# AlexIoannides/bodywork-mlops-demo

Measured on NVIDIA H100. Metric: train rows/sec (N x 128 least-squares fit), higher is better.
Workload: dtype bf16x2 (hi+lo) MMA operands, f32 accumulate, f64 fold+solve

## Files before the change

bodywork-mlops-demo_b200/csrc/solve.cu:

```cuda
#include "b2_internal.cuh"
#include "b2_xchg.cuh"

namespace b2 {
namespace {

constexpr int kOutIntercept = kMaxD;
constexpr int kOutInfo = kMaxD + 1;
constexpr int kOutRank = kMaxD + 2;
constexpr int kOutSingular = kMaxD + 3;
constexpr int kOutRows = kOutSingular + kMaxD;

struct LdcgStat {
  const double* S;
  __device__ __forceinline__ double operator()(int i) const { return __ldcg(S + i); }
};

template <class Stat>
__device__ void build_normal_equations_of(const Stat& S, int d, double alpha, int fit_intercept,
                                       double* A, double* r, double* mean, double* ybar_out) {
  const int dp = d + 2, pitch = d + 1;
  const double n = S(d * dp + d);
  const double inv_n = n > 0.0 ? 1.0 / n : 0.0;
  double sxy = 0.0;
  if ((int)threadIdx.x < d) {
    const double sx = S(threadIdx.x * dp + d);
    sxy = S(threadIdx.x * dp + d + 1);
    mean[threadIdx.x] = fit_intercept ? sx * inv_n : 0.0;
  }
  const double ybar = fit_intercept ? S(d * dp + d + 1) * inv_n : 0.0;
  __syncthreads();
  if ((int)threadIdx.x < d) r[threadIdx.x] = sxy - n * mean[threadIdx.x] * ybar;
  const int lane = threadIdx.x & 31, warp = threadIdx.x >> 5, nwarps = blockDim.x >> 5;
  for (int i0 = warp; i0 < d; i0 += 2 * nwarps) {
    const int i1 = i0 + nwarps;
    double v[8];
#pragma unroll
    for (int u = 0; u < 4; ++u) {
      const int j = lane + 32 * u;
      v[u] = j < d ? S(i0 * dp + j) : 0.0;
      v[4 + u] = (j < d && i1 < d) ? S(i1 * dp + j) : 0.0;
    }
    const double m0 = mean[i0], m1 = i1 < d ? mean[i1] : 0.0;
#pragma unroll
    for (int u = 0; u < 4; ++u) {
      const int j = lane + 32 * u;
      if (j < d) {
        const double mj = mean[j];
        A[i0 * pitch + j] = v[u] - n * m0 * mj + (i0 == j ? alpha : 0.0);
        if (i1 < d) A[i1 * pitch + j] = v[4 + u] - n * m1 * mj + (i1 == j ? alpha : 0.0);
      }
    }
  }
  if (threadIdx.x == 0) *ybar_out = ybar;
  __syncthreads();
}

__device__ __forceinline__ void build_normal_equations(const double* S, int d, double alpha, int fit_intercept,
                                                       double* A, double* r, double* mean, double* ybar_out) {
  build_normal_equations_of(LdcgStat{S}, d, alpha, fit_intercept, A, r, mean, ybar_out);
}

__device__ __forceinline__ double rcp_pos(double x) {
  double y;
  asm("rcp.approx.ftz.f64 %0, %1;" : "=d"(y) : "d"(x));
  const double er = fma(-x, y, 1.0);
  const double t = fma(er, er, er);
  return fma(y, t, y);
}

struct SolveXchg {
  double* own;
  int n_ranks;
  unsigned int epoch;
  unsigned long long timeout_ns;
};

constexpr int kNB = 16;
constexpr int kCholThreads = 512;
constexpr int kUPitch = kNB + 1;

__device__ void refine_update(const double* S, int d, int fit_intercept, bool singular, const double* dbeta, double* misc,
                              double* __restrict__ rf, double* __restrict__ out);

template <bool REFINE>
__global__ void __launch_bounds__(kCholThreads, 1)
solve_cholesky_kernel(double* S, int d, double alpha, int fit_intercept, double* __restrict__ out, const SolveXchg xc,
                      double* __restrict__ rf) {
  extern __shared__ double sm[];
  const int pitch = d + 1;
  double* A = sm;
  double* r = A + d * pitch;
  double* mean = A + (d + 1) * pitch;
  double* invd = mean + d;
  double* misc = invd + d;
  double* U = misc + 8;
  const int tid = threadIdx.x, lane = tid & 31;
  const int warp = __shfl_sync(0xffffffffu, tid >> 5, 0);
  long long tm[5] = {0, 0, 0, 0, 0};
  long long tc0 = clock64();
  if (xc.own != nullptr) {
    __shared__ int ok;
    if (tid == 0) ok = xchg_wait(xc.own, xc.n_ranks, xc.epoch, xc.timeout_ns) ? 1 : 0;
    __syncthreads();
    if (!ok) {
      if (tid == 0) {
        xchg_flags(xc.own)[kXchgStatusWord] = xc.epoch;
        out[kOutInfo] = -1.0;
      }
      return;
    }
    const int dp = d + 2;
    for (int base = 0; base < dp * dp; base += 4 * blockDim.x) {
      double sv[4];
#pragma unroll
      for (int u = 0; u < 4; ++u) {
        const int idx = base + u * blockDim.x + tid;
        sv[u] = idx < dp * dp ? xchg_sum(xc.own, xc.n_ranks, xc.epoch, idx) : 0.0;
      }
#pragma unroll
      for (int u = 0; u < 4; ++u) {
        const int idx = base + u * blockDim.x + tid;
        if (idx < dp * dp) S[idx] = sv[u];
      }
    }
    __threadfence();
    __syncthreads();
  }
  build_normal_equations(S, d, alpha, fit_intercept, A, r, mean, &misc[0]);
  if constexpr (REFINE) {
    if (tid < d) r[tid] = rf[kRfGrad + tid] - alpha * rf[kRfBeta + tid];
    __syncthreads();
  }
  tm[0] = clock64() - tc0;
  if (warp == 0) {
    double mx = 0.0;
    for (int i = lane; i < d; i += 32) mx = fmax(mx, A[i * pitch + i]);
#pragma unroll
    for (int o = 16; o > 0; o >>= 1) mx = fmax(mx, __shfl_xor_sync(0xffffffffu, mx, o));
    if (lane == 0) { misc[1] = mx; misc[2] = 0.0; }
  }
  __syncthreads();
  const double tiny = misc[1] * 1e-12;
  const int rows = d + 1;

  for (int kb = 0; kb < d; kb += kNB) {
    const int nb = (d - kb) < kNB ? (d - kb) : kNB;
    tc0 = clock64();
    if (warp == 0) {
      const int lrow = lane & (kNB - 1), h = lane >> 4;
      const bool act = lrow < nb;
      const int row = kb + (act ? lrow : 0);
      double a[kNB / 2];
#pragma unroll
      for (int cc = 0; cc < kNB / 2; ++cc) {
        const int c = 2 * cc + h;
        a[cc] = (act && c < nb) ? A[row * pitch + kb + c] : 0.0;
      }
      double my_rc = 1.0;
      int first_bad = 0;
#pragma unroll
      for (int k = 0; k < kNB; ++k) {
        if (k < nb) {
          const int hk = k & 1, kk = k >> 1;
          const double colk = a[kk];
          const double piv = __shfl_sync(0xffffffffu, colk, k | (hk << 4));
          const bool bad = !(piv > tiny);
          const double rc = bad ? 1.0 : rcp_pos(piv);
          const double u = __shfl_sync(0xffffffffu, colk, lrow | (hk << 4));
          my_rc = (lrow == k) ? rc : my_rc;
          first_bad = (bad && first_bad == 0) ? (kb + k + 1) : first_bad;
#pragma unroll
          for (int cc = 0; cc < kNB / 2; ++cc) {
            if (2 * cc + 1 > k) {
              const int c = 2 * cc + h;
              const double uc = __shfl_sync(0xffffffffu, colk, c | (hk << 4));
              if (c > k) a[cc] = fma(-(u * uc), rc, a[cc]);
            }
          }
          if (h == hk && act && lrow > k) {
            A[row * pitch + kb + k] = u * rc;
            U[row * kUPitch + k] = u;
          }
        }
      }
      if (act && h == 0) invd[kb + lrow] = my_rc;
      if (lane == 0 && first_bad != 0 && misc[2] == 0.0) misc[2] = (double)first_bad;
    }
    __syncthreads();
    tm[1] += clock64() - tc0; tc0 = clock64();
    if (misc[2] != 0.0) break;
    {
      const int prow = tid >> 2, q = tid & 3;
      const int below = rows - kb - nb;
      const bool live = prow < below;
      const int i = kb + nb + (live ? prow : 0);
      double sv[4];
#pragma unroll
      for (int j = 0; j < 4; ++j) {
        const int c = 4 * j + q;
        sv[j] = (live && c < nb) ? A[i * pitch + kb + c] : 0.0;
      }
      const int qbase = lane & ~3;
      double rinv[kNB];
#pragma unroll
      for (int m = 0; m < kNB; ++m) rinv[m] = m < nb ? invd[kb + m] : 0.0;
      double out_m[4], out_u[4];
#pragma unroll
      for (int j = 0; j < 4; ++j) { out_m[j] = 0.0; out_u[j] = 0.0; }
#pragma unroll
      for (int m = 0; m < kNB; ++m) {
        if (m < nb) {
          const double um = __shfl_sync(0xffffffffu, sv[m >> 2], qbase | (m & 3));
          const double xm = um * rinv[m];
          if (q == (m & 3)) { out_m[m >> 2] = xm; out_u[m >> 2] = um; }
#pragma unroll
          for (int j = 0; j < 4; ++j) {
            if (4 * j + 3 > m) {
              const int c = 4 * j + q;
              if (c > m && c < nb) sv[j] = fma(-xm, U[(kb + c) * kUPitch + m], sv[j]);
            }
          }
        }
      }
      if (live) {
#pragma unroll
        for (int j = 0; j < 4; ++j) {
          const int m = 4 * j + q;
          if (m < nb) { A[i * pitch + kb + m] = out_m[j]; U[i * kUPitch + m] = out_u[j]; }
        }
      }
    }
    __syncthreads();
    tm[2] += clock64() - tc0; tc0 = clock64();
    {
      const int base = kb + nb;
      const int nti = (rows - base + 7) >> 3, ntj = (d - base + 7) >> 3;
      const int tri = ntj * (ntj + 1) / 2;
      const int total = tri + (nti > ntj ? ntj : 0);
      const int g = lane >> 2, t4 = lane & 3;
      constexpr int kWarps = kCholThreads / 32, kInFlight = 4;
      for (int t0 = warp; t0 < total; t0 += kWarps * kInFlight) {
        int ia[kInFlight], jb[kInFlight];
        double c0[kInFlight], c1[kInFlight], av[kInFlight][kNB / 4], bv[kInFlight][kNB / 4];
#pragma unroll
        for (int f = 0; f < kInFlight; ++f) {
          const int t = t0 + f * kWarps;
          int ti = 0, tj = 0;
          if (t < tri) {
            ti = (int)((sqrtf(8.0f * (float)t + 1.0f) - 1.0f) * 0.5f);
            while (ti * (ti + 1) / 2 > t) --ti;
            while ((ti + 1) * (ti + 2) / 2 <= t) ++ti;
            tj = t - ti * (ti + 1) / 2;
          } else if (t < total) {
            ti = ntj; tj = t - tri;
          }
          const bool live = t < total;
          ia[f] = live ? base + 8 * ti + g : rows;
          jb[f] = live ? base + 8 * tj + g : d;
#pragma unroll
          for (int sgm = 0; sgm < kNB / 4; ++sgm) {
            const int m = 4 * sgm + t4;
            av[f][sgm] = (ia[f] < rows && m < nb) ? -A[ia[f] * pitch + kb + m] : 0.0;
            bv[f][sgm] = (jb[f] < d && m < nb) ? U[jb[f] * kUPitch + m] : 0.0;
          }
          c0[f] = 0.0; c1[f] = 0.0;
        }
#pragma unroll
        for (int sgm = 0; sgm < kNB / 4; ++sgm) {
#pragma unroll
          for (int f = 0; f < kInFlight; ++f)
            asm volatile("mma.sync.aligned.m8n8k4.row.col.f64.f64.f64.f64 {%0, %1}, {%2}, {%3}, {%0, %1};"
                         : "+d"(c0[f]), "+d"(c1[f]) : "d"(av[f][sgm]), "d"(bv[f][sgm]));
        }
#pragma unroll
        for (int f = 0; f < kInFlight; ++f) {
          const int jc = jb[f] - g + 2 * t4;
          if (ia[f] < rows) {
            if (jc < d) A[ia[f] * pitch + jc] += c0[f];
            if (jc + 1 < d) A[ia[f] * pitch + jc + 1] += c1[f];
          }
        }
      }
    }
    __syncthreads();
    tm[3] += clock64() - tc0;
  }
  tc0 = clock64();
  const bool singular = misc[2] != 0.0;
  if (!singular) {
    for (int kb = ((d - 1) / kNB) * kNB; kb >= 0; kb -= kNB) {
      const int nb = (d - kb) < kNB ? (d - kb) : kNB;
      if (warp == 0) {
        const int col = lane & (kNB - 1);
        const bool act = lane < nb;
        double lt[kNB];
#pragma unroll
        for (int k = 0; k < kNB; ++k) lt[k] = (act && k < nb && k > col) ? A[(kb + k) * pitch + kb + col] : 0.0;
        double z = act ? r[kb + col] : 0.0;
#pragma unroll
        for (int k = kNB - 1; k >= 0; --k) {
          if (k < nb) {
            const double bk = __shfl_sync(0xffffffffu, z, k);
            z = (lane < k) ? fma(-lt[k], bk, z) : z;
          }
        }
        __syncwarp();
        if (act) r[kb + lane] = z;
      }
      __syncthreads();
      for (int i = tid; i < kb; i += blockDim.x) {
        double acc0 = 0.0, acc1 = 0.0;
#pragma unroll
        for (int m = 0; m < kNB; m += 2) {
          if (m < nb) acc0 = fma(A[(kb + m) * pitch + i], r[kb + m], acc0);
          if (m + 1 < nb) acc1 = fma(A[(kb + m + 1) * pitch + i], r[kb + m + 1], acc1);
        }
        r[i] -= acc0 + acc1;
      }
      __syncthreads();
    }
  }
  tm[4] = clock64() - tc0;
  if constexpr (REFINE) {
    refine_update(S, d, fit_intercept, singular, r, misc, rf, out);
    return;
  }
  if (tid == 0)
    for (int k = 0; k < 5; ++k) out[kOutSingular + k] = (double)tm[k];
  for (int i = tid; i < d; i += blockDim.x) out[i] = singular ? 0.0 : r[i];
  if (warp == 0) {
    double part = 0.0;
    for (int i = lane; i < d; i += 32) part += mean[i] * r[i];
#pragma unroll
    for (int o = 16; o > 0; o >>= 1) part += __shfl_xor_sync(0xffffffffu, part, o);
    if (lane == 0) {
      out[kOutIntercept] = singular ? 0.0 : misc[0] - part;
      out[kOutInfo] = misc[2];
    }
  }
}

__device__ void refine_update(const double* S, int d, int fit_intercept, bool singular, const double* dbeta, double* misc,
                              double* __restrict__ rf, double* __restrict__ out) {
  const int tid = threadIdx.x, lane = tid & 31, warp = tid >> 5;
  const int dp = d + 2;
  const double n = __ldcg(S + d * dp + d);
  if (warp == 0) {
    double mx = 0.0;
    bool finite = true;
    for (int i = lane; i < d; i += 32) {
      const double sx = __ldcg(S + i * dp + d);
      const double c = __ldcg(S + i * dp + i) - sx * (sx / n);
      mx = fmax(mx, fabs(dbeta[i]) * sqrt(fmax(c, 0.0)));
      finite = finite && isfinite(dbeta[i]);
    }
#pragma unroll
    for (int o = 16; o > 0; o >>= 1) mx = fmax(mx, __shfl_xor_sync(0xffffffffu, mx, o));
    finite = __all_sync(0xffffffffu, finite) && isfinite(rf[kRfGrad + kMaxD]);
    if (lane == 0) {
      const double sy = __ldcg(S + d * dp + d + 1);
      const double cy = __ldcg(S + (d + 1) * dp + d + 1) - sy * (sy / n);
      const double sig = sqrt(fmax(cy, 0.0));
      const double step = sig > 0.0 ? mx / sig : mx;
      misc[3] = step;
      misc[4] = (singular || !finite || !(step <= rf[kRfStep])) ? 1.0 : 0.0;
    }
  }
  __syncthreads();
  const bool guard = misc[4] != 0.0;
  for (int i = tid; i < d; i += blockDim.x) {
    const double b = rf[kRfBeta + i];
    if (guard) {
      rf[kRfBeta + i] = rf[kRfPrevBeta + i];
    } else {
      rf[kRfPrevBeta + i] = b;
      rf[kRfBeta + i] = b + dbeta[i];
    }
  }
  if (tid == 0) {
    const double b0 = rf[kRfB0];
    if (guard) {
      rf[kRfB0] = rf[kRfPrevB0];
    } else {
      rf[kRfPrevB0] = b0;
      rf[kRfB0] = fit_intercept ? b0 + rf[kRfGrad + kMaxD] / n : b0;
      rf[kRfStep] = misc[3];
    }
  }
  __syncthreads();
  for (int i = tid; i < d; i += blockDim.x) out[i] = rf[kRfBeta + i];
  if (warp == 0) {
    double part = 0.0;
    for (int i = lane; i < d; i += 32) part += rf[kRfMean + i] * rf[kRfBeta + i];
#pragma unroll
    for (int o = 16; o > 0; o >>= 1) part += __shfl_xor_sync(0xffffffffu, part, o);
    if (lane == 0) {
      out[kOutIntercept] = rf[kRfB0] - part;
      out[kOutInfo] = misc[2];
      out[kOutRefineStep] = misc[3];
      out[kOutRefineGuard] = misc[4];
    }
  }
}

__device__ __forceinline__ void rr_pair(int m, int round, int k, int* p, int* q) {
  const int mm = m - 1;
  int a, b;
  if (k == 0) { a = mm; b = round % mm; }
  else { a = (round + k) % mm; b = (round - k + mm) % mm; }
  *p = a < b ? a : b;
  *q = a < b ? b : a;
}

__global__ void __launch_bounds__(512, 1)
solve_spectral_kernel(const double* __restrict__ S, int d, double cond, int fit_intercept,
                      double* __restrict__ out) {
  extern __shared__ double sm[];
  const int pitch = d + 1;
  double* W = sm;
  double* r = W + d * pitch;
  double* mean = r + d;
  double* lam = mean + d;
  double* misc = lam + d;
  __shared__ int rotated;
  build_normal_equations(S, d, 0.0, fit_intercept, W, r, mean, &misc[0]);

  const int m = d + (d & 1);
  const int pairs = m / 2;
  const int sub = threadIdx.x & 7;
  const int slot0 = threadIdx.x >> 3;
  for (int sweep = 0; sweep < 24 && d > 1; ++sweep) {
    if (threadIdx.x == 0) rotated = 0;
    __syncthreads();
    for (int round = 0; round < m - 1; ++round) {
      for (int slot = slot0; slot < ((pairs + 63) / 64) * 64; slot += 64) {
        int p = 0, q = 0;
        const bool live_slot = slot < pairs;
        if (live_slot) rr_pair(m, round, slot, &p, &q);
        const bool live = live_slot && q < d;
        double a = 0.0, b = 0.0, g = 0.0;
        if (live) {
          for (int row = sub; row < d; row += 8) {
            const double wp = W[p * pitch + row], wq = W[q * pitch + row];
            a += wp * wp; b += wq * wq; g += wp * wq;
          }
        }
#pragma unroll
        for (int o = 1; o < 8; o <<= 1) {
          a += __shfl_xor_sync(0xffffffffu, a, o);
          b += __shfl_xor_sync(0xffffffffu, b, o);
          g += __shfl_xor_sync(0xffffffffu, g, o);
        }
        if (live && fabs(g) > 1e-15 * sqrt(a * b) && a * b > 0.0) {
          const double zeta = (b - a) / (2.0 * g);
          const double t = (zeta >= 0.0 ? 1.0 : -1.0) / (fabs(zeta) + sqrt(1.0 + zeta * zeta));
          const double c = 1.0 / sqrt(1.0 + t * t), s = c * t;
          for (int row = sub; row < d; row += 8) {
            const double wp = W[p * pitch + row], wq = W[q * pitch + row];
            W[p * pitch + row] = c * wp - s * wq;
            W[q * pitch + row] = s * wp + c * wq;
          }
          if (sub == 0 && fabs(g) > 1e-13 * sqrt(a * b)) rotated = 1;
        }
      }
      __syncthreads();
    }
    if (!rotated) break;
    __syncthreads();
  }
  {
// ... 1177 lines not shown
```

bodywork-mlops-demo_b200/csrc/gram_tc.cu:

```cuda
#include <cuda_bf16.h>
#include <stdlib.h>

#include "b2_internal.cuh"
#include "b2_ptx.cuh"
#include "b2_shift.cuh"
#include "b2_xchg.cuh"

namespace b2 {
namespace {

constexpr int kConsumerWGs = 2;
constexpr int kXformWarps = 8;
constexpr int kThreads = 128 * (kConsumerWGs + 2);
constexpr int kFirstXformWarp = 4 * kConsumerWGs;
constexpr int kTmaWarp = kFirstXformWarp;
constexpr int kEWarp = kFirstXformWarp + 1;
static_assert(kFirstXformWarp + kXformWarps == kThreads / 32, "warp roles");
constexpr int kProducers = kXformWarps;
constexpr int kConsumerWarps = 4 * kConsumerWGs;
constexpr int kKGroups = kTcRows / 8;
constexpr uint32_t kRawStageBytes = kTcRows * kMaxD * 4;
constexpr uint32_t kOpSBO = 128;
constexpr uint32_t kOpLBO = (16 + 2 + 16) * kOpSBO;
constexpr uint32_t kOpEOff = 16 * kOpSBO;
constexpr uint32_t kOpLoOff = 18 * kOpSBO;
constexpr uint32_t kOpStageBytes = kKGroups * kOpLBO;
constexpr int kMaxPack = 5;
constexpr uint32_t kYStageBytes = kTcRows * kMaxPack * 4;
constexpr uint32_t kMStageBytes = 384;
static_assert(kMStageBytes >= kTcRows * kMaxPack && kMStageBytes % 128 == 0 && kYStageBytes % 128 == 0, "stage alignment");

template <bool RAWB>
struct TcGeo {
  static constexpr int kRawStages = RAWB ? 4 : 3;
  static constexpr int kOpStages = RAWB ? 2 : 3;
  static constexpr int kAhead = RAWB ? kRawStages - 2 : kRawStages - 1;
  static constexpr uint32_t kOffRaw = 0;
  static constexpr uint32_t kOffOp = kOffRaw + kRawStages * kRawStageBytes;
  static constexpr uint32_t kOffY = kOffOp + kOpStages * kOpStageBytes;
  static constexpr uint32_t kOffMask = kOffY + kRawStages * kYStageBytes;
  static constexpr uint32_t kOffBar = kOffMask + kRawStages * kMStageBytes;
  static constexpr int kNumBars = 2 * kRawStages + 2 * kOpStages;
  static constexpr uint32_t kOffShift = kOffBar + kNumBars * 8;
  static constexpr uint32_t kOffESum = kOffShift + (kMaxD + 4) * 4;
  static constexpr uint32_t kSmemBytes = kOffESum + 3 * 32 * 8 + 1024;
  static_assert(kSmemBytes <= 227 * 1024, "shared memory budget");
  static constexpr uint32_t kConsumerRegs = RAWB ? 200 : 192, kProducerRegs = RAWB ? 56 : 64;
  static_assert(kConsumerRegs * 128 * kConsumerWGs + kProducerRegs * (kThreads - 128 * kConsumerWGs) <= 65536,
                "register budget");
};

constexpr uint64_t kEvictFirst = 0x12F0000000000000ull;

__device__ __forceinline__ void tma_load_2d(uint32_t dst, const CUtensorMap* tm, int c0, int c1, uint32_t bar) {
  asm volatile(
      "cp.async.bulk.tensor.2d.shared::cluster.global.mbarrier::complete_tx::bytes.L2::cache_hint"
      " [%0], [%1, {%3, %4}], [%2], %5;" ::"r"(dst),
      "l"(reinterpret_cast<uint64_t>(tm)), "r"(bar), "r"(c0), "r"(c1), "l"(kEvictFirst)
      : "memory");
}
__device__ __forceinline__ void tma_load_1d(uint32_t dst, const CUtensorMap* tm, int c0, uint32_t bar) {
  asm volatile(
      "cp.async.bulk.tensor.1d.shared::cluster.global.mbarrier::complete_tx::bytes.L2::cache_hint"
      " [%0], [%1, {%3}], [%2], %4;" ::"r"(dst),
      "l"(reinterpret_cast<uint64_t>(tm)), "r"(bar), "r"(c0), "l"(kEvictFirst)
      : "memory");
}
__device__ __forceinline__ void tma_prefetch_desc(const CUtensorMap* tm) {
  asm volatile("prefetch.tensormap [%0];" ::"l"(reinterpret_cast<uint64_t>(tm)) : "memory");
}

__device__ __forceinline__ uint64_t make_smem_desc(uint32_t addr) {
  return (uint64_t)((addr & 0x3FFFFu) >> 4) | ((uint64_t)(kOpLBO >> 4) << 16) | ((uint64_t)(kOpSBO >> 4) << 32);
}
__device__ __forceinline__ void wgmma_fence() { asm volatile("wgmma.fence.sync.aligned;" ::: "memory"); }
__device__ __forceinline__ void wgmma_commit() { asm volatile("wgmma.commit_group.sync.aligned;" ::: "memory"); }
template <int N>
__device__ __forceinline__ void wgmma_wait() { asm volatile("wgmma.wait_group.sync.aligned %0;" ::"n"(N) : "memory"); }
template <int N>
__device__ __forceinline__ void fence_regs(float (&r)[N]) {
#pragma unroll
  for (int i = 0; i < N; ++i) asm volatile("" : "+f"(r[i])::"memory");
}
template <int N, int TB>
__device__ __forceinline__ void wgmma(float* d, uint64_t adesc, uint64_t bdesc, uint32_t scale_d);
#define B2_ACC4(o) "+f"(d[o]), "+f"(d[o + 1]), "+f"(d[o + 2]), "+f"(d[o + 3])
#define B2_ACC8(o) B2_ACC4(o), B2_ACC4(o + 4)
template <>
__device__ __forceinline__ void wgmma<8, 0>(float* d, uint64_t adesc, uint64_t bdesc, uint32_t scale_d) {
  asm volatile(
      "{\n\t.reg .pred p;\n\tsetp.ne.b32 p, %6, 0;\n\t"
      "wgmma.mma_async.sync.aligned.m64n8k16.f32.bf16.bf16 "
      "{%0, %1, %2, %3}, "
      "%4, %5, p, 1, 1, 0, 0;\n\t}"
      : B2_ACC4(0)
      : "l"(adesc), "l"(bdesc), "r"(scale_d));
}
template <>
__device__ __forceinline__ void wgmma<72, 0>(float* d, uint64_t adesc, uint64_t bdesc, uint32_t scale_d) {
  asm volatile(
      "{\n\t.reg .pred p;\n\tsetp.ne.b32 p, %38, 0;\n\t"
      "wgmma.mma_async.sync.aligned.m64n72k16.f32.bf16.bf16 "
      "{%0, %1, %2, %3, %4, %5, %6, %7, %8, %9, %10, %11, %12, %13, %14, %15, "
      "%16, %17, %18, %19, %20, %21, %22, %23, %24, %25, %26, %27, %28, %29, %30, %31, "
      "%32, %33, %34, %35}, "
      "%36, %37, p, 1, 1, 0, 0;\n\t}"
      : B2_ACC8(0), B2_ACC8(8), B2_ACC8(16), B2_ACC8(24), B2_ACC4(32)
      : "l"(adesc), "l"(bdesc), "r"(scale_d));
}
template <>
__device__ __forceinline__ void wgmma<80, 0>(float* d, uint64_t adesc, uint64_t bdesc, uint32_t scale_d) {
  asm volatile(
      "{\n\t.reg .pred p;\n\tsetp.ne.b32 p, %42, 0;\n\t"
      "wgmma.mma_async.sync.aligned.m64n80k16.f32.bf16.bf16 "
      "{%0, %1, %2, %3, %4, %5, %6, %7, %8, %9, %10, %11, %12, %13, %14, %15, "
      "%16, %17, %18, %19, %20, %21, %22, %23, %24, %25, %26, %27, %28, %29, %30, %31, "
      "%32, %33, %34, %35, %36, %37, %38, %39}, "
      "%40, %41, p, 1, 1, 0, 0;\n\t}"
      : B2_ACC8(0), B2_ACC8(8), B2_ACC8(16), B2_ACC8(24), B2_ACC8(32)
      : "l"(adesc), "l"(bdesc), "r"(scale_d));
}
template <>
__device__ __forceinline__ void wgmma<136, 0>(float* d, uint64_t adesc, uint64_t bdesc, uint32_t scale_d) {
  asm volatile(
      "{\n\t.reg .pred p;\n\tsetp.ne.b32 p, %70, 0;\n\t"
      "wgmma.mma_async.sync.aligned.m64n136k16.f32.bf16.bf16 "
      "{%0, %1, %2, %3, %4, %5, %6, %7, %8, %9, %10, %11, %12, %13, %14, %15, "
      "%16, %17, %18, %19, %20, %21, %22, %23, %24, %25, %26, %27, %28, %29, %30, %31, "
      "%32, %33, %34, %35, %36, %37, %38, %39, %40, %41, %42, %43, %44, %45, %46, %47, "
      "%48, %49, %50, %51, %52, %53, %54, %55, %56, %57, %58, %59, %60, %61, %62, %63, "
      "%64, %65, %66, %67}, "
      "%68, %69, p, 1, 1, 0, 0;\n\t}"
      : B2_ACC8(0), B2_ACC8(8), B2_ACC8(16), B2_ACC8(24), B2_ACC8(32), B2_ACC8(40), B2_ACC8(48), B2_ACC8(56), B2_ACC4(64)
      : "l"(adesc), "l"(bdesc), "r"(scale_d));
}
template <>
__device__ __forceinline__ void wgmma<144, 0>(float* d, uint64_t adesc, uint64_t bdesc, uint32_t scale_d) {
  asm volatile(
      "{\n\t.reg .pred p;\n\tsetp.ne.b32 p, %74, 0;\n\t"
      "wgmma.mma_async.sync.aligned.m64n144k16.f32.bf16.bf16 "
      "{%0, %1, %2, %3, %4, %5, %6, %7, %8, %9, %10, %11, %12, %13, %14, %15, "
      "%16, %17, %18, %19, %20, %21, %22, %23, %24, %25, %26, %27, %28, %29, %30, %31, "
      "%32, %33, %34, %35, %36, %37, %38, %39, %40, %41, %42, %43, %44, %45, %46, %47, "
      "%48, %49, %50, %51, %52, %53, %54, %55, %56, %57, %58, %59, %60, %61, %62, %63, "
      "%64, %65, %66, %67, %68, %69, %70, %71}, "
      "%72, %73, p, 1, 1, 0, 0;\n\t}"
      : B2_ACC8(0), B2_ACC8(8), B2_ACC8(16), B2_ACC8(24), B2_ACC8(32), B2_ACC8(40), B2_ACC8(48), B2_ACC8(56), B2_ACC8(64)
      : "l"(adesc), "l"(bdesc), "r"(scale_d));
}
template <>
__device__ __forceinline__ void wgmma<64, 1>(float* d, uint64_t adesc, uint64_t bdesc, uint32_t scale_d) {
  asm volatile(
      "{\n\t.reg .pred p;\n\tsetp.ne.b32 p, %34, 0;\n\t"
      "wgmma.mma_async.sync.aligned.m64n64k16.f32.bf16.bf16 "
      "{%0, %1, %2, %3, %4, %5, %6, %7, %8, %9, %10, %11, %12, %13, %14, %15, "
      "%16, %17, %18, %19, %20, %21, %22, %23, %24, %25, %26, %27, %28, %29, %30, %31}, "
      "%32, %33, p, 1, 1, 0, 1;\n\t}"
      : B2_ACC8(0), B2_ACC8(8), B2_ACC8(16), B2_ACC8(24)
      : "l"(adesc), "l"(bdesc), "r"(scale_d));
}
template <>
__device__ __forceinline__ void wgmma<128, 1>(float* d, uint64_t adesc, uint64_t bdesc, uint32_t scale_d) {
  asm volatile(
      "{\n\t.reg .pred p;\n\tsetp.ne.b32 p, %66, 0;\n\t"
      "wgmma.mma_async.sync.aligned.m64n128k16.f32.bf16.bf16 "
      "{%0, %1, %2, %3, %4, %5, %6, %7, %8, %9, %10, %11, %12, %13, %14, %15, "
      "%16, %17, %18, %19, %20, %21, %22, %23, %24, %25, %26, %27, %28, %29, %30, %31, "
      "%32, %33, %34, %35, %36, %37, %38, %39, %40, %41, %42, %43, %44, %45, %46, %47, "
      "%48, %49, %50, %51, %52, %53, %54, %55, %56, %57, %58, %59, %60, %61, %62, %63}, "
      "%64, %65, p, 1, 1, 0, 1;\n\t}"
      : B2_ACC8(0), B2_ACC8(8), B2_ACC8(16), B2_ACC8(24), B2_ACC8(32), B2_ACC8(40), B2_ACC8(48), B2_ACC8(56)
      : "l"(adesc), "l"(bdesc), "r"(scale_d));
}
#undef B2_ACC8
#undef B2_ACC4
constexpr uint32_t kRawBoxBytes = kTcRows * 64 * 2;
__device__ __forceinline__ uint64_t make_raw_desc(uint32_t addr) {
  return (uint64_t)((addr & 0x3FFFFu) >> 4) | ((uint64_t)(kRawBoxBytes >> 4) << 16) | ((uint64_t)(1024u >> 4) << 32) |
         (1ull << 62);
}

__device__ __forceinline__ void st_shared_v4(uint32_t addr, const uint32_t (&v)[4]) {
  asm volatile("st.shared.v4.b32 [%0], {%1, %2, %3, %4};" ::"r"(addr), "r"(v[0]), "r"(v[1]), "r"(v[2]), "r"(v[3])
               : "memory");
}
__device__ __forceinline__ uint32_t lane_id() {
  uint32_t l;
  asm volatile("mov.u32 %0, %%laneid;" : "=r"(l));
  return l;
}
__device__ __forceinline__ void st_shared_f64(uint32_t addr, double v) {
  asm volatile("st.shared.f64 [%0], %1;" ::"r"(addr), "d"(v) : "memory");
}
__device__ __forceinline__ double ld_shared_f64(uint32_t addr) {
  double v;
  asm volatile("ld.shared.f64 %0, [%1];" : "=d"(v) : "r"(addr) : "memory");
  return v;
}
__device__ __forceinline__ void put_f64(double* p, double v, bool add, bool on) {
  if (add)
    asm volatile("{\n\t.reg .pred p;\n\tsetp.ne.b32 p, %2, 0;\n\t@p red.global.add.f64 [%0], %1;\n\t}"
                 ::"l"(p), "d"(v), "r"((uint32_t)on) : "memory");
  else
    asm volatile("{\n\t.reg .pred p;\n\tsetp.ne.b32 p, %2, 0;\n\t@p st.global.f64 [%0], %1;\n\t}"
                 ::"l"(p), "d"(v), "r"((uint32_t)on) : "memory");
}
__device__ __forceinline__ void st_shared_u16(uint32_t addr, uint32_t v) {
  asm volatile("st.shared.u16 [%0], %1;" ::"r"(addr), "h"((unsigned short)v) : "memory");
}
__device__ __forceinline__ void split2(float v0, float v1, uint32_t& hi, uint32_t& lo) {
  const __nv_bfloat162 h = __floats2bfloat162_rn(v0, v1);
  hi = *reinterpret_cast<const uint32_t*>(&h);
  const float h0 = __uint_as_float(hi << 16), h1 = __uint_as_float(hi & 0xffff0000u);
  const __nv_bfloat162 l = __floats2bfloat162_rn(v0 - h0, v1 - h1);
  lo = *reinterpret_cast<const uint32_t*>(&l);
}

constexpr int kRedElems = kTcAccElems + kTcSums;

__device__ __forceinline__ void tc_reduce_range(const double* part, int n_ctas, int n_acc, double* red, int e0, int e1,
                                                double* quarter) {
  const int epb = blockDim.x >> 2;
  const int e = threadIdx.x % epb, q = threadIdx.x / epb;
  const int per = (n_ctas + 3) / 4;
  const int c0 = q * per, c1 = (c0 + per < n_ctas) ? c0 + per : n_ctas;
  for (int base = e0; base < e1; base += epb) {
    const int idx = base + e;
    const bool sum = idx >= n_acc;
    if (idx < e1) {
      const double* src = sum ? part + (size_t)n_ctas * kTcAccElems + (idx - n_acc) : part + idx;
      const size_t stride = sum ? kTcSums : kTcAccElems;
      double acc[8] = {0.0, 0.0, 0.0, 0.0, 0.0, 0.0, 0.0, 0.0};
      int c = c0;
      for (; c + 8 <= c1; c += 8) {
#pragma unroll
        for (int u = 0; u < 8; ++u) acc[u] += __ldcg(src + (size_t)(c + u) * stride);
      }
      for (; c < c1; ++c) acc[0] += __ldcg(src + (size_t)c * stride);
      quarter[q * epb + e] = ((acc[0] + acc[1]) + (acc[2] + acc[3])) + ((acc[4] + acc[5]) + (acc[6] + acc[7]));
    }
    __syncthreads();
    if (q == 0 && idx < e1)
      red[sum ? kTcAccElems + (idx - n_acc) : idx] =
          ((quarter[e] + quarter[epb + e]) + quarter[2 * epb + e]) + quarter[3 * epb + e];
    __syncthreads();
  }
}

__device__ __forceinline__ void grid_barrier(unsigned int* ctr) {
  __syncthreads();
  if (threadIdx.x == 0) {
    __threadfence();
    atomicAdd(ctr, 1u);
    const uint64_t t0 = globaltimer_ns();
    unsigned int seen;
    do {
      asm volatile("ld.acquire.gpu.global.u32 %0, [%1];" : "=r"(seen) : "l"(ctr) : "memory");
      if (seen < gridDim.x) {
        __nanosleep(40);
        if (globaltimer_ns() - t0 > 4000000000ull) __trap();
      }
    } while (seen < gridDim.x);
    __threadfence();
  }
  __syncthreads();
}

__device__ __forceinline__ double tc_fold_value(const double* red, const double* c, int d, int pack, int ew, bool d2,
                                                int idx) {
  const int dp = d + 2;
  const int a = min(idx / dp, idx % dp), b = max(idx / dp, idx % dp);
  auto P = [&](int acc, int i, int j) { return __ldcg(red + tc_part_index(acc, i, j, ew)); };
  auto s1 = [&](int i) {
    double t = 0.0;
    for (int blk = 0; blk < pack; ++blk) {
      const int r = blk * d + i, e = kTcM + 3 * blk;
      t += d2 ? P(0, r, e) + P(1, r, e) : P(0, r, e);
    }
    return t;
  };
  auto sxy = [&](int i) {
    double t = 0.0;
    for (int blk = 0; blk < pack; ++blk) {
      const int r = blk * d + i, e = kTcM + 3 * blk;
      t += d2 ? P(0, r, e + 1) + P(0, r, e + 2) + P(1, r, e + 1) + P(1, r, e + 2) : P(0, r, e + 1) + P(0, r, e + 2);
    }
    return t;
  };
  auto G = [&](int i, int j) {
    double g = 0.0;
    for (int blk = 0; blk < pack; ++blk) {
      const int ia = blk * d + i, ib = blk * d + j;
      const double g1 = P(0, min(ia, ib), max(ia, ib));
      g += d2 ? g1 + P(1, ia, ib) + P(1, ib, ia) : g1;
    }
    return g;
  };
  return unshift_entry(a, b, d, c, G, s1, sxy, __ldcg(red + kTcAccElems + 2), __ldcg(red + kTcAccElems + 0),
                       __ldcg(red + kTcAccElems + 1));
}

template <typename T, int DFIX, bool SPLIT, bool RAWB = false, int EW = 8>
__global__ void __launch_bounds__(kThreads, 1)
gram_tc_kernel(const __grid_constant__ CUtensorMap tmX, const __grid_constant__ CUtensorMap tmY,
               const __grid_constant__ CUtensorMap tmM, int y_map_2d, int has_mask, int keep,
               int64_t n_rows, int d_arg, int pack, int d_orig, const float* __restrict__ shift,
               int chunk_tiles, double* __restrict__ part, uint32_t wait_ns, uint32_t dbg_arg) {
#ifdef B2_DEV_KNOBS
  const uint32_t dbg = dbg_arg;
#else
  constexpr uint32_t dbg = 0u;
  (void)dbg_arg;
#endif
  using G = TcGeo<RAWB>;
  constexpr int kRawStages = G::kRawStages, kOpStages = G::kOpStages;
  constexpr uint32_t kOffRaw = G::kOffRaw, kOffOp = G::kOffOp, kOffY = G::kOffY, kOffMask = G::kOffMask;
  const int d = DFIX ? DFIX : d_arg;
  extern __shared__ uint8_t smem_raw[];
  const uint32_t sbase = (smem_u32(smem_raw) + 1023u) & ~1023u;
  uint8_t* smem = smem_raw + (sbase - smem_u32(smem_raw));
  const int warp = threadIdx.x >> 5;
  const int lane = threadIdx.x & 31;

  const uint32_t bar_raw_full = sbase + G::kOffBar;
  const uint32_t bar_raw_empty = bar_raw_full + 8 * kRawStages;
  const uint32_t bar_op_full = bar_raw_empty + 8 * kRawStages;
  const uint32_t bar_op_empty = bar_op_full + 8 * kOpStages;
  float* shift_s = reinterpret_cast<float*>(smem + G::kOffShift);

  const int64_t total_tiles = (n_rows + kTcRows - 1) / kTcRows;
  const int64_t tile_begin = (int64_t)blockIdx.x * total_tiles / gridDim.x;
  const int64_t tile_end = (int64_t)(blockIdx.x + 1) * total_tiles / gridDim.x;
  const int my_tiles = (int)(tile_end - tile_begin);

  if (threadIdx.x == 0) {
    for (int s = 0; s < kRawStages; ++s) {
      mbar_init(bar_raw_full + 8 * s, 1);
      mbar_init(bar_raw_empty + 8 * s, kProducers + (RAWB ? kConsumerWarps : 0));
    }
    for (int s = 0; s < kOpStages; ++s) {
      mbar_init(bar_op_full + 8 * s, kProducers);
      mbar_init(bar_op_empty + 8 * s, kConsumerWarps);
    }
    asm volatile("fence.mbarrier_init.release.cluster;" ::: "memory");
  }
  if (warp == kTmaWarp && lane == 0) {
    tma_prefetch_desc(&tmX);
    tma_prefetch_desc(&tmY);
    if (has_mask) tma_prefetch_desc(&tmM);
  }
  for (uint32_t o = threadIdx.x * 16; o < kOpStages * kOpStageBytes; o += kThreads * 16)
    *reinterpret_cast<uint4*>(smem + kOffOp + o) = make_uint4(0, 0, 0, 0);
  for (int j = threadIdx.x; j <= kMaxD; j += kThreads)
    shift_s[j] = j == kMaxD ? shift[kMaxD] : (j < pack * d_orig ? shift[j % d_orig] : 0.f);
  fence_proxy_async_smem();
  __syncthreads();

  if (warp < kConsumerWarps) {
    asm volatile("setmaxnreg.inc.sync.aligned.u32 %0;" ::"n"(G::kConsumerRegs));
    auto consume = [&](auto wg_c) {
      constexpr int WG = decltype(wg_c)::value;
      constexpr int kF1 = kTcM - 64 * WG;
      constexpr int kF2 = RAWB ? kF1 : kTcM;
      constexpr int kC1 = 64 * WG;
      constexpr int kR1 = (kF1 + EW) / 2, kR2 = (kF2 + EW) / 2;
      float acc1[kR1], acc2[kR2];
      double* my_part = part + (size_t)blockIdx.x * kTcAccElems;
      auto store = [&](auto n_regs, int dst_acc, int col0, bool add, auto val) {
        const int ln = (int)lane_id(), row0 = 64 * WG + 16 * (warp & 3) + (ln >> 2);
#pragma unroll
        for (int r = 0; r < decltype(n_regs)::value; ++r) {
          const int col = col0 + 8 * (r >> 2) + 2 * (ln & 3) + (r & 1), h = (r >> 1) & 1, i = row0 + 8 * h;
          const bool lower = dst_acc == 0 && col < kTcM && i > col;
          put_f64(my_part + tc_part_index(dst_acc, i, col, EW), val(r, col, h), add, !lower);
        }
      };
      auto drain = [&](const auto& acc, int dst_acc, int col0, bool add) {
        constexpr int kR = sizeof(acc) / sizeof(float);
        if constexpr (RAWB) {
          constexpr int kF = 2 * kR - EW;
          const double s1[2] = {(double)__shfl_sync(0xffffffffu, acc[kF / 2], lane & ~3),
                                (double)__shfl_sync(0xffffffffu, acc[kF / 2 + 2], lane & ~3)};
          store(std::integral_constant<int, kR>{}, dst_acc, col0, add, [&](int r, int col, int h) {
            return col < kTcM ? (double)acc[r] - (double)shift_s[col] * s1[h] : (double)acc[r];
          });
        } else {
          store(std::integral_constant<int, kR>{}, dst_acc, col0, add, [&](int r, int, int) { return (double)acc[r]; });
        }
      };
      auto release = [&](int tile) {
        mbar_arrive(bar_op_empty + 8 * (tile % kOpStages));
        if constexpr (RAWB) mbar_arrive(bar_raw_empty + 8 * (tile % kRawStages));
      };
      constexpr uint32_t a_off = (uint32_t)WG * 8 * kOpSBO;
      int os = 0, held = -1, in_chunk = 0;
      uint32_t oph = 0;
      bool first_chunk = true;
      for (int it = 0; it < my_tiles; ++it) {
        mbar_wait(bar_op_full + 8 * os, oph, wait_ns);
        const uint32_t op_addr = sbase + kOffOp + os * kOpStageBytes;
        wgmma_fence();
#pragma unroll
        for (int k2 = 0; k2 < kTcRows / 16; ++k2) {
          const uint32_t k_addr = op_addr + k2 * 2 * kOpLBO;
          const uint64_t hi_desc = make_smem_desc(k_addr + a_off), lo_desc = make_smem_desc(k_addr + kOpLoOff + a_off);
          const uint32_t sc1 = (in_chunk > 0 || k2 > 0) ? 1u : 0u, sc2 = (it > 0 || k2 > 0) ? 1u : 0u;
          if constexpr (RAWB) {
            const uint64_t x_desc = make_raw_desc(sbase + kOffRaw + (uint32_t)(it % kRawStages) * kRawStageBytes +
                                                  (uint32_t)WG * kRawBoxBytes + k2 * 16 * 128);
            const uint64_t e_desc = make_smem_desc(k_addr + kOpEOff);
            if (!(dbg & 2u)) {
              wgmma<kF1, 1>(acc1, hi_desc, x_desc, sc1);
              wgmma<EW, 0>(acc1 + kF1 / 2, hi_desc, e_desc, sc1);
            }
            if (SPLIT && !(dbg & 3u)) {
              wgmma<kF2, 1>(acc2, lo_desc, x_desc, sc2);
              wgmma<EW, 0>(acc2 + kF2 / 2, lo_desc, e_desc, sc2);
            }
          } else {
            if (!(dbg & 2u)) wgmma<kF1 + EW, 0>(acc1, hi_desc, make_smem_desc(k_addr + a_off), sc1);
            if (SPLIT && !(dbg & 3u)) wgmma<kF2 + EW, 0>(acc2, lo_desc, make_smem_desc(k_addr), sc2);
          }
        }
        wgmma_commit();
        const bool last = (in_chunk == chunk_tiles - 1) || (it == my_tiles - 1);
        if (last) {
          wgmma_wait<0>();
          fence_regs(acc1);
          if constexpr (SPLIT) fence_regs(acc2);
        } else {
          wgmma_wait<1>();
        }
        if (lane == 0) {
          if (held >= 0) release(held);
          if (last) release(it);
        }
        held = last ? -1 : it;
        if (last) {
          drain(acc1, 0, kC1, !first_chunk);
          first_chunk = false;
          in_chunk = 0;
        } else {
          ++in_chunk;
        }
        if (++os == kOpStages) { os = 0; oph ^= 1; }
      }
      wgmma_wait<0>();
      if constexpr (SPLIT) {
        fence_regs(acc2);
        drain(acc2, RAWB ? 0 : 1, RAWB ? kC1 : 0, RAWB);
      }
    };
    if (__shfl_sync(0xffffffffu, warp, 0) >= 4) consume(std::integral_constant<int, 1>{});
    else consume(std::integral_constant<int, 0>{});
  } else {
    asm volatile("setmaxnreg.dec.sync.aligned.u32 %0;" ::"n"(G::kProducerRegs));
    const uint32_t tx = (uint32_t)(kTcRows * d * sizeof(T)) + kTcRows * pack * 4 + (has_mask ? kTcRows * pack : 0);
    auto issue = [&](int j) {
      const int s = j % kRawStages;
      mbar_wait(bar_raw_empty + 8 * s, ((uint32_t)(j / kRawStages) & 1u) ^ 1u, wait_ns);
      const uint32_t full = bar_raw_full + 8 * s;
      mbar_expect_tx(full, tx);
      const int64_t row0 = (tile_begin + j) * kTcRows;
      tma_load_2d(sbase + kOffRaw + s * kRawStageBytes, &tmX, 0, (int)row0, full);
      if constexpr (RAWB) tma_load_2d(sbase + kOffRaw + s * kRawStageBytes + kRawBoxBytes, &tmX, 64, (int)row0, full);
      const int sub0 = (int)row0 * pack;
      if (y_map_2d) tma_load_2d(sbase + kOffY + s * kYStageBytes, &tmY, 0, sub0 >> 2, full);
      else tma_load_1d(sbase + kOffY + s * kYStageBytes, &tmY, sub0, full);
      if (has_mask == 2) tma_load_2d(sbase + kOffMask + s * kMStageBytes, &tmM, 0, sub0 >> 4, full);
      else if (has_mask) tma_load_1d(sbase + kOffMask + s * kMStageBytes, &tmM, sub0, full);
    };
    const bool issuer = warp == kTmaWarp && lane == 0;
    if (issuer)
      for (int j = 0; j < G::kAhead && j < my_tiles; ++j) issue(j);

    const int t = warp - kFirstXformWarp;
    const int nb = (d + 63) >> 6;
    const int i = 64 * (t % nb) + 2 * lane;
    const uint32_t swp = ((uint32_t)lane >> 2) & 1u;
    const uint32_t st_off = (uint32_t)((i >> 3) * kOpSBO + (i & 7) * 16);
    auto esum = [&]() { return sbase + G::kOffESum + 8 * lane_id(); };
    if (warp == kEWarp) { st_shared_f64(esum(), 0.0); st_shared_f64(esum() + 256, 0.0); st_shared_f64(esum() + 512, 0.0); }
    int rs = 0, os = 0;
    uint32_t rph = 0, oph = 0;
    for (int it = 0; it < my_tiles; ++it) {
      if (issuer && it + G::kAhead < my_tiles) issue(it + G::kAhead);
      __syncwarp();
      mbar_wait(bar_raw_full + 8 * rs, rph, wait_ns);
      mbar_wait(bar_op_empty + 8 * os, oph ^ 1, wait_ns);
      const int64_t row0 = (tile_begin + it) * kTcRows;
      const int64_t left = n_rows - row0;
      const int rows_valid = left < kTcRows ? (int)left : kTcRows;
      const bool full_tile = (!has_mask) && (rows_valid == kTcRows);
      const uint32_t raw_addr = sbase + kOffRaw + rs * kRawStageBytes;
      const uint32_t m_addr = sbase + kOffMask + rs * kMStageBytes;
      const uint32_t op_addr = sbase + kOffOp + os * kOpStageBytes;
      if (warp == kEWarp && !(dbg & 192u)) {
        const uint32_t y_addr = sbase + kOffY + rs * kYStageBytes;
        const uint32_t e_addr = op_addr + kOpEOff;
        const float c_y = shift_s[kMaxD];
        float a = 0.f, b = 0.f, c = 0.f;
        for (int half = 0; half < kTcRows / 32; ++half) {
          const int rr = lane + 32 * half;
          const uint32_t dst = e_addr + (rr >> 3) * kOpLBO + (rr & 7) * 2;
          for (int bl = 0; bl < pack; ++bl) {
            const int sub = rr * pack + bl;
            bool use = rr < rows_valid;
            if (use && has_mask) use = (ld_shared_u8(m_addr + sub) == (uint32_t)keep);
            const float yv = use ? ld_shared_f32(y_addr + sub * 4) - c_y : 0.f;
            uint32_t yh, yl;
            split2(yv, 0.f, yh, yl);
            st_shared_u16(dst + (3 * bl) * 16, use ? 0x3F80u : 0u);
            st_shared_u16(dst + (3 * bl + 1) * 16, yh);
            st_shared_u16(dst + (3 * bl + 2) * 16, yl);
            if (RAWB && has_mask && !use) {
              const uint32_t row = raw_addr + (uint32_t)rr * 128;
              const uint32_t z[4] = {0u, 0u, 0u, 0u};
#pragma unroll
              for (int q = 0; q < 8; ++q) { st_shared_v4(row + 16 * q, z); st_shared_v4(row + kRawBoxBytes + 16 * q, z); }
            }
            a += yv;
            b = fmaf(yv, yv, b);
            c += use ? 1.f : 0.f;
          }
        }
        const uint32_t es = esum();
        st_shared_f64(es, ld_shared_f64(es) + (double)a);
        st_shared_f64(es + 256, ld_shared_f64(es + 256) + (double)b);
        st_shared_f64(es + 512, ld_shared_f64(es + 512) + (double)c);
      }
      if (i < d && !(dbg & 128u)) {
        float c_i[2];
        ld_vals_vec<float, 2>(sbase + G::kOffShift + 4 * (uint32_t)i, c_i);
        for (int g = t / nb; g < kKGroups; g += kXformWarps / nb) {
          const int r0 = g * 8;
          float v0[8], v1[8];
          const uint32_t src = raw_addr + (uint32_t)r0 * ((uint32_t)d * sizeof(T)) + (uint32_t)i * sizeof(T);
#pragma unroll
          for (int k = 0; k < 8; ++k) {
            const uint32_t a = RAWB ? raw_addr + (uint32_t)(i >> 6) * kRawBoxBytes + (uint32_t)(r0 + k) * 128 +
                                          ((((uint32_t)(i & 63) >> 3) ^ (uint32_t)k) << 4) + (uint32_t)(i & 7) * 2
                                    : src + (uint32_t)k * ((uint32_t)d * sizeof(T));
            float x[2];
            if (dbg & 8u) { x[0] = __uint_as_float(src + k); x[1] = __uint_as_float(src - k); }
            else ld_vals_vec<T, 2>(a, x);
            v0[k] = x[0] - c_i[0];
            v1[k] = x[1] - c_i[1];
          }
          if (!full_tile) {
            const int blk = i / d_orig;
#pragma unroll
            for (int k = 0; k < 8; ++k) {
              bool use = (r0 + k) < rows_valid;
              if (use && has_mask) use = (ld_shared_u8(m_addr + (r0 + k) * pack + blk) == (uint32_t)keep);
              if (!use) { v0[k] = 0.f; v1[k] = 0.f; }
            }
          }
          uint32_t h0[4], l0[4], h1[4], l1[4];
#pragma unroll
          for (int p = 0; p < 4; ++p) {
            if constexpr (SPLIT) {
              split2(v0[2 * p], v0[2 * p + 1], h0[p], l0[p]);
              split2(v1[2 * p], v1[2 * p + 1], h1[p], l1[p]);
            } else {
              const __nv_bfloat162 e0 = __floats2bfloat162_rn(v0[2 * p], v0[2 * p + 1]);
              const __nv_bfloat162 e1 = __floats2bfloat162_rn(v1[2 * p], v1[2 * p + 1]);
              h0[p] = *reinterpret_cast<const uint32_t*>(&e0);
              h1[p] = *reinterpret_cast<const uint32_t*>(&e1);
              l0[p] = l1[p] = 0u;
            }
          }
          if (!(dbg & 4u)) {
            const uint32_t dst = op_addr + (uint32_t)g * kOpLBO + st_off;
            uint32_t f[4], s[4];
#pragma unroll
            for (int p = 0; p < 4; ++p) { f[p] = swp ? h1[p] : h0[p]; s[p] = swp ? h0[p] : h1[p]; }
            st_shared_v4(dst + 16 * swp, f);
            st_shared_v4(dst + 16 - 16 * swp, s);
            if constexpr (SPLIT) {
#pragma unroll
              for (int p = 0; p < 4; ++p) { f[p] = swp ? l1[p] : l0[p]; s[p] = swp ? l0[p] : l1[p]; }
              st_shared_v4(dst + kOpLoOff + 16 * swp, f);
              st_shared_v4(dst + kOpLoOff + 16 - 16 * swp, s);
            }
          }
        }
      }
      if (!(dbg & 32u)) fence_proxy_async_smem();
      __syncwarp();
      if (lane == 0) {
        mbar_arrive(bar_op_full + 8 * os);
        mbar_arrive(bar_raw_empty + 8 * rs);
      }
      if (++rs == kRawStages) { rs = 0; rph ^= 1; }
      if (++os == kOpStages) { os = 0; oph ^= 1; }
    }
    if (warp == kEWarp) {
      const uint32_t es = esum();
      double sy = ld_shared_f64(es), syy = ld_shared_f64(es + 256), cnt = ld_shared_f64(es + 512);
#pragma unroll
      for (int o = 16; o > 0; o >>= 1) {
        sy += __shfl_xor_sync(0xffffffffu, sy, o);
        syy += __shfl_xor_sync(0xffffffffu, syy, o);
        cnt += __shfl_xor_sync(0xffffffffu, cnt, o);
// ... 266 lines not shown
```

Before: 5.418 billion.

## Overlap back-substitution sweeps with diagonal solve and prefetch normal-equation rows

The back-substitution loop is restructured so that warp 0 first updates the next diagonal block's rows from the previous block's solution and then solves that block. Meanwhile, the other warps sweep the remaining rows with the lagged update. This removes one __syncthreads per block. Separately, the statistic loads for the first rows in build_normal_equations are issued before the mean and ybar computation and barrier, which hides their latency. The cost is more complex lag-by-one bookkeeping, and one warp is left out of the bulk sweep.

```diff
diff --git a/bodywork-mlops-demo_b200/csrc/solve.cu b/bodywork-mlops-demo_b200/csrc/solve.cu
--- a/bodywork-mlops-demo_b200/csrc/solve.cu
+++ b/bodywork-mlops-demo_b200/csrc/solve.cu
@@ -19,35 +19,45 @@
 __device__ void build_normal_equations_of(const Stat& S, int d, double alpha, int fit_intercept,
                                        double* A, double* r, double* mean, double* ybar_out) {
   const int dp = d + 2, pitch = d + 1;
+  const int lane = threadIdx.x & 31, warp = threadIdx.x >> 5, nwarps = blockDim.x >> 5;
+  constexpr int kRows = 2;
+  double v[kRows][4];
+  auto load_rows = [&](int i0) {
+#pragma unroll
+    for (int k = 0; k < kRows; ++k) {
+      const int i = i0 + k * nwarps;
+#pragma unroll
+      for (int u = 0; u < 4; ++u) {
+        const int j = lane + 32 * u;
+        v[k][u] = (j < d && i < d) ? S(i * dp + j) : 0.0;
+      }
+    }
+  };
   const double n = S(d * dp + d);
+  double sx = 0.0, sxy = 0.0;
+  if ((int)threadIdx.x < d) {
+    sx = S(threadIdx.x * dp + d);
+    sxy = S(threadIdx.x * dp + d + 1);
+  }
+  const double sy = S(d * dp + d + 1);
+  load_rows(warp);
   const double inv_n = n > 0.0 ? 1.0 / n : 0.0;
-  double sxy = 0.0;
-  if ((int)threadIdx.x < d) {
-    const double sx = S(threadIdx.x * dp + d);
-    sxy = S(threadIdx.x * dp + d + 1);
-    mean[threadIdx.x] = fit_intercept ? sx * inv_n : 0.0;
-  }
-  const double ybar = fit_intercept ? S(d * dp + d + 1) * inv_n : 0.0;
+  if ((int)threadIdx.x < d) mean[threadIdx.x] = fit_intercept ? sx * inv_n : 0.0;
+  const double ybar = fit_intercept ? sy * inv_n : 0.0;
   __syncthreads();
   if ((int)threadIdx.x < d) r[threadIdx.x] = sxy - n * mean[threadIdx.x] * ybar;
-  const int lane = threadIdx.x & 31, warp = threadIdx.x >> 5, nwarps = blockDim.x >> 5;
-  for (int i0 = warp; i0 < d; i0 += 2 * nwarps) {
-    const int i1 = i0 + nwarps;
-    double v[8];
-#pragma unroll
-    for (int u = 0; u < 4; ++u) {
-      const int j = lane + 32 * u;
-      v[u] = j < d ? S(i0 * dp + j) : 0.0;
-      v[4 + u] = (j < d && i1 < d) ? S(i1 * dp + j) : 0.0;
-    }
-    const double m0 = mean[i0], m1 = i1 < d ? mean[i1] : 0.0;
-#pragma unroll
-    for (int u = 0; u < 4; ++u) {
-      const int j = lane + 32 * u;
-      if (j < d) {
-        const double mj = mean[j];
-        A[i0 * pitch + j] = v[u] - n * m0 * mj + (i0 == j ? alpha : 0.0);
-        if (i1 < d) A[i1 * pitch + j] = v[4 + u] - n * m1 * mj + (i1 == j ? alpha : 0.0);
+  for (int i0 = warp; i0 < d; i0 += kRows * nwarps) {
+    if (i0 != warp) load_rows(i0);
+#pragma unroll
+    for (int k = 0; k < kRows; ++k) {
+      const int i = i0 + k * nwarps;
+      if (i < d) {
+        const double mi = mean[i];
+#pragma unroll
+        for (int u = 0; u < 4; ++u) {
+          const int j = lane + 32 * u;
+          if (j < d) A[i * pitch + j] = v[k][u] - n * mi * mean[j] + (i == j ? alpha : 0.0);
+        }
       }
     }
   }
@@ -288,34 +298,42 @@
   tc0 = clock64();
   const bool singular = misc[2] != 0.0;
   if (!singular) {
-    for (int kb = ((d - 1) / kNB) * kNB; kb >= 0; kb -= kNB) {
+    auto solve_block = [&](int kb) {
       const int nb = (d - kb) < kNB ? (d - kb) : kNB;
+      const int col = lane & (kNB - 1);
+      const bool act = lane < nb;
+      double lt[kNB];
+#pragma unroll
+      for (int k = 0; k < kNB; ++k) lt[k] = (act && k < nb && k > col) ? A[(kb + k) * pitch + kb + col] : 0.0;
+      double z = act ? r[kb + col] : 0.0;
+#pragma unroll
+      for (int k = kNB - 1; k >= 0; --k) {
+        if (k < nb) {
+          const double bk = __shfl_sync(0xffffffffu, z, k);
+          z = (lane < k) ? fma(-lt[k], bk, z) : z;
+        }
+      }
+      __syncwarp();
+      if (act) r[kb + lane] = z;
+    };
+    auto sweep_row = [&](int i, int kb) {
+      const int nb = (d - kb) < kNB ? (d - kb) : kNB;
+      double acc0 = 0.0, acc1 = 0.0;
+#pragma unroll
+      for (int m = 0; m < kNB; m += 2) {
+        if (m < nb) acc0 = fma(A[(kb + m) * pitch + i], r[kb + m], acc0);
+        if (m + 1 < nb) acc1 = fma(A[(kb + m + 1) * pitch + i], r[kb + m + 1], acc1);
+      }
+      r[i] -= acc0 + acc1;
+    };
+    const int kb_last = ((d - 1) / kNB) * kNB;
+    for (int kb = kb_last; kb >= 0; kb -= kNB) {
       if (warp == 0) {
-        const int col = lane & (kNB - 1);
-        const bool act = lane < nb;
-        double lt[kNB];
-#pragma unroll
-        for (int k = 0; k < kNB; ++k) lt[k] = (act && k < nb && k > col) ? A[(kb + k) * pitch + kb + col] : 0.0;
-        double z = act ? r[kb + col] : 0.0;
-#pragma unroll
-        for (int k = kNB - 1; k >= 0; --k) {
-          if (k < nb) {
-            const double bk = __shfl_sync(0xffffffffu, z, k);
-            z = (lane < k) ? fma(-lt[k], bk, z) : z;
-          }
-        }
+        if (kb != kb_last && lane < kNB) sweep_row(kb + lane, kb + kNB);
         __syncwarp();
-        if (act) r[kb + lane] = z;
-      }
-      __syncthreads();
-      for (int i = tid; i < kb; i += blockDim.x) {
-        double acc0 = 0.0, acc1 = 0.0;
-#pragma unroll
-        for (int m = 0; m < kNB; m += 2) {
-          if (m < nb) acc0 = fma(A[(kb + m) * pitch + i], r[kb + m], acc0);
-          if (m + 1 < nb) acc1 = fma(A[(kb + m + 1) * pitch + i], r[kb + m + 1], acc1);
-        }
-        r[i] -= acc0 + acc1;
+        solve_block(kb);
+      } else if (kb != kb_last) {
+        for (int i = tid - 32; i < kb; i += blockDim.x - 32) sweep_row(i, kb + kNB);
       }
       __syncthreads();
     }
```

After: 5.367 billion, median of 6. No clear change (-0.9%).

## Keep per-chunk fp64 partial sums on chip instead of global red.add

Applied to the files above, without the earlier changes.

Consumer warps now accumulate part of their per-chunk fp64 partial Gram results in registers or in a new shared-memory slab, instead of issuing red.global.add.f64 for every chunk drain. A single flush writes these sums to global at the end. This targets global atomic traffic and latency during drains. In exchange it uses more registers and shared memory and adds a debug switch that disables the on-chip path.

```diff
diff --git a/bodywork-mlops-demo_b200/csrc/gram_tc.cu b/bodywork-mlops-demo_b200/csrc/gram_tc.cu
--- a/bodywork-mlops-demo_b200/csrc/gram_tc.cu
+++ b/bodywork-mlops-demo_b200/csrc/gram_tc.cu
@@ -43,11 +43,25 @@
   static constexpr int kNumBars = 2 * kRawStages + 2 * kOpStages;
   static constexpr uint32_t kOffShift = kOffBar + kNumBars * 8;
   static constexpr uint32_t kOffESum = kOffShift + (kMaxD + 4) * 4;
-  static constexpr uint32_t kSmemBytes = kOffESum + 3 * 32 * 8 + 1024;
+  static constexpr int kSlabSlots = RAWB ? 22 : 21;
+  static constexpr uint32_t kOffSlab = kOffESum + 3 * 32 * 8;
+  static constexpr uint32_t kSmemBytes = kOffSlab + kSlabSlots * 4 * 32 * 8 + 1024;
   static_assert(kSmemBytes <= 227 * 1024, "shared memory budget");
   static constexpr uint32_t kConsumerRegs = RAWB ? 200 : 192, kProducerRegs = RAWB ? 56 : 64;
   static_assert(kConsumerRegs * 128 * kConsumerWGs + kProducerRegs * (kThreads - 128 * kConsumerWGs) <= 65536,
                 "register budget");
+};
+
+template <int DFIX, bool SPLIT, bool RAWB, int EW, int WG>
+struct TcSums {
+  static constexpr int kR1 = (kTcM - 64 * WG + EW) / 2;
+  static constexpr bool kTight = SPLIT && !RAWB && (EW == 16 || DFIX == 0);
+  static constexpr int kRegs = WG == 1 ? (kTight ? (EW == 16 ? 24 : 28) : kR1)
+                                       : (!SPLIT ? 40 : (RAWB || EW == 16 ? 0 : (DFIX ? 16 : 8)));
+  static constexpr int kSlab = WG == 1 ? 0 : TcGeo<RAWB>::kSlabSlots;
+  static constexpr int kSlabBase = WG == 1 ? TcSums<DFIX, SPLIT, RAWB, EW, 0>::kSlab : 0;
+  static constexpr int kFirstSlab = kR1 - kRegs - kSlab, kFirstReg = kR1 - kRegs;
+  static_assert(kFirstSlab >= 0 && kSlabBase + kSlab <= TcGeo<RAWB>::kSlabSlots, "fp64 sum homes");
 };
 
 constexpr uint64_t kEvictFirst = 0x12F0000000000000ull;
@@ -204,6 +218,10 @@
   else
     asm volatile("{\n\t.reg .pred p;\n\tsetp.ne.b32 p, %2, 0;\n\t@p st.global.f64 [%0], %1;\n\t}"
                  ::"l"(p), "d"(v), "r"((uint32_t)on) : "memory");
+}
+__device__ __forceinline__ void st_shared_f64_if(uint32_t addr, double v, bool on) {
+  asm volatile("{\n\t.reg .pred p;\n\tsetp.ne.b32 p, %2, 0;\n\t@p st.shared.f64 [%0], %1;\n\t}"
+               ::"r"(addr), "d"(v), "r"((uint32_t)on) : "memory");
 }
 __device__ __forceinline__ void st_shared_u16(uint32_t addr, uint32_t v) {
   asm volatile("st.shared.u16 [%0], %1;" ::"r"(addr), "h"((unsigned short)v) : "memory");
@@ -365,14 +383,38 @@
       constexpr int kC1 = 64 * WG;
       constexpr int kR1 = (kF1 + EW) / 2, kR2 = (kF2 + EW) / 2;
       float acc1[kR1], acc2[kR2];
+      using H = TcSums<DFIX, SPLIT, RAWB, EW, WG>;
       double* my_part = part + (size_t)blockIdx.x * kTcAccElems;
+      double sums[H::kRegs > 0 ? H::kRegs : 1];
+      const bool on_chip_off = (dbg & 256u) != 0u;
+      auto slab_addr = [&](int s, int ln) {
+        return sbase + G::kOffSlab + (uint32_t)(((4 * H::kSlabBase + (warp & 3) * H::kSlab + s) * 32 + ln) * 8);
+      };
       auto store = [&](auto n_regs, int dst_acc, int col0, bool add, auto val) {
         const int ln = (int)lane_id(), row0 = 64 * WG + 16 * (warp & 3) + (ln >> 2);
 #pragma unroll
         for (int r = 0; r < decltype(n_regs)::value; ++r) {
           const int col = col0 + 8 * (r >> 2) + 2 * (ln & 3) + (r & 1), h = (r >> 1) & 1, i = row0 + 8 * h;
           const bool lower = dst_acc == 0 && col < kTcM && i > col;
-          put_f64(my_part + tc_part_index(dst_acc, i, col, EW), val(r, col, h), add, !lower);
+          const double v = val(r, col, h);
+          const bool on_chip = dst_acc == 0 && r >= H::kFirstSlab;
+          if (on_chip && r >= H::kFirstReg) {
+            double& s = sums[r - H::kFirstReg];
+            s = add ? __dadd_rn(s, v) : v;
+          } else if (on_chip) {
+            const uint32_t a = slab_addr(r - H::kFirstSlab, ln);
+            st_shared_f64_if(a, add ? __dadd_rn(ld_shared_f64(a), v) : v, !on_chip_off);
+          }
+          put_f64(my_part + tc_part_index(dst_acc, i, col, EW), v, add, !lower && (!on_chip || on_chip_off));
+        }
+      };
+      auto flush = [&]() {
+        const int ln = (int)lane_id(), row0 = 64 * WG + 16 * (warp & 3) + (ln >> 2);
+#pragma unroll
+        for (int r = H::kFirstSlab; r < H::kR1; ++r) {
+          const int col = kC1 + 8 * (r >> 2) + 2 * (ln & 3) + (r & 1), i = row0 + 8 * ((r >> 1) & 1);
+          const double s = r >= H::kFirstReg ? sums[r - H::kFirstReg] : ld_shared_f64(slab_addr(r - H::kFirstSlab, ln));
+          put_f64(my_part + tc_part_index(0, i, col, EW), s, false, !(col < kTcM && i > col) && !on_chip_off);
         }
       };
       auto drain = [&](const auto& acc, int dst_acc, int col0, bool add) {
@@ -450,6 +492,7 @@
         fence_regs(acc2);
         drain(acc2, RAWB ? 0 : 1, RAWB ? kC1 : 0, RAWB);
       }
+      flush();
     };
     if (__shfl_sync(0xffffffffu, warp, 0) >= 4) consume(std::integral_constant<int, 1>{});
     else consume(std::integral_constant<int, 0>{});
```

Result: faster. 5.297 billion before, 5.506 billion after (median of 6 runs) (+3.9%).
